# sczhou/CodeFormer

Hardware: NVIDIA H100
Metric: faces_per_sec_512x512_batch32 (higher is better)
Workload: dtype f32 (split-fp16 operands on tensor cores, fp32 accumulate)

## Files before the change

### codeformer_b200/csrc/simt_kernels.cu

```cuda
#include <cuda_fp16.h>
#include <cuda_runtime.h>

#include <atomic>
#include <math.h>
#include <stdint.h>

#include "kernels.cuh"

namespace cfb {

__device__ __forceinline__ float silu_f(float x) { return x / (1.f + expf(-x)); }
__device__ __forceinline__ float gelu_f(float x) { return 0.5f * x * (1.f + erff(x * 0.70710678118654752440f)); }
__device__ __forceinline__ float lrelu_f(float x) { return x > 0.f ? x : 0.2f * x; }

constexpr int CF_BM = 128;
constexpr int CF_BK = 16;
constexpr int CF_APITCH = CF_BM + 4;

template <int BN>
__global__ void __launch_bounds__(256) conv_f32_kernel(ConvArgs a) {
  constexpr int TN = BN / 16;
  __shared__ __align__(16) float As[2][CF_BK][CF_APITCH];
  __shared__ __align__(16) float Bs[2][CF_BK][BN];

  const int t = threadIdx.x;
  const int64_t M = (int64_t)a.N * a.Ho * a.Wo;
  const int64_t m0 = (int64_t)blockIdx.x * CF_BM;
  const int n0 = blockIdx.y * BN;
  const int taps = a.ksize * a.ksize;
  const int kchunks = a.Cin / CF_BK;
  const int nk = taps * kchunks;

  const int arow = t >> 1;
  const int akq = (t & 1) * 8;
  const int64_t am = m0 + arow;
  const bool arow_ok = am < M;
  int an = 0, aoy = 0, aox = 0;
  if (arow_ok) {
    an = (int)(am / ((int64_t)a.Ho * a.Wo));
    int rem = (int)(am - (int64_t)an * a.Ho * a.Wo);
    aoy = rem / a.Wo;
    aox = rem - aoy * a.Wo;
  }
  const float* in_n = a.in + (int64_t)an * a.H * a.W * a.Cin;
  const float* sc_n = a.in_scale ? a.in_scale + (int64_t)an * a.Cin : nullptr;
  const float* sh_n = a.in_shift ? a.in_shift + (int64_t)an * a.Cin : nullptr;

  constexpr int BV = (CF_BK * BN / 4) / 256;
  const int bcol = (BN == 128) ? (t & 31) * 4 : (t & 15) * 4;
  const int brow0 = (BN == 128) ? (t >> 5) : (t >> 4);

  float4 ra[2], rb[BV];

  auto load_global = [&](int it) {
    const int tap = it / kchunks;
    const int c0 = (it - tap * kchunks) * CF_BK;
    int r = 0, s = 0;
    if (a.ksize == 3) { r = tap / 3; s = tap - r * 3; }
    bool ok = arow_ok;
    int iy, ix;
    if (a.mode == CONV_DOWN) {
      iy = aoy * 2 + r; ix = aox * 2 + s;
      ok = ok && iy < a.H && ix < a.W;
    } else if (a.mode == CONV_UP) {
      iy = aoy + r - 1; ix = aox + s - 1;
      ok = ok && iy >= 0 && ix >= 0 && iy < 2 * a.H && ix < 2 * a.W;
      iy >>= 1; ix >>= 1;
    } else {
      const int p = a.ksize >> 1;
      iy = aoy + r - p; ix = aox + s - p;
      ok = ok && iy >= 0 && ix >= 0 && iy < a.H && ix < a.W;
    }
    if (ok) {
      const float* p = in_n + ((int64_t)iy * a.W + ix) * a.Cin + c0 + akq;
      ra[0] = __ldg(reinterpret_cast<const float4*>(p));
      ra[1] = __ldg(reinterpret_cast<const float4*>(p + 4));
      if (sc_n) {
        const float4 s0 = __ldg(reinterpret_cast<const float4*>(sc_n + c0 + akq));
        const float4 s1 = __ldg(reinterpret_cast<const float4*>(sc_n + c0 + akq + 4));
        const float4 h0 = __ldg(reinterpret_cast<const float4*>(sh_n + c0 + akq));
        const float4 h1 = __ldg(reinterpret_cast<const float4*>(sh_n + c0 + akq + 4));
        ra[0].x = fmaf(ra[0].x, s0.x, h0.x); ra[0].y = fmaf(ra[0].y, s0.y, h0.y);
        ra[0].z = fmaf(ra[0].z, s0.z, h0.z); ra[0].w = fmaf(ra[0].w, s0.w, h0.w);
        ra[1].x = fmaf(ra[1].x, s1.x, h1.x); ra[1].y = fmaf(ra[1].y, s1.y, h1.y);
        ra[1].z = fmaf(ra[1].z, s1.z, h1.z); ra[1].w = fmaf(ra[1].w, s1.w, h1.w);
      }
      if (a.in_act == IN_SILU) {
        ra[0].x = silu_f(ra[0].x); ra[0].y = silu_f(ra[0].y); ra[0].z = silu_f(ra[0].z); ra[0].w = silu_f(ra[0].w);
        ra[1].x = silu_f(ra[1].x); ra[1].y = silu_f(ra[1].y); ra[1].z = silu_f(ra[1].z); ra[1].w = silu_f(ra[1].w);
      }
    } else {
      ra[0] = make_float4(0.f, 0.f, 0.f, 0.f);
      ra[1] = ra[0];
    }
    const float* wb = a.wgt_f32 + ((int64_t)tap * a.Cin + c0) * a.Cout + n0 + bcol;
#pragma unroll
    for (int i = 0; i < BV; ++i) {
      const int kr = brow0 + i * 8;
      rb[i] = __ldg(reinterpret_cast<const float4*>(wb + (int64_t)kr * a.Cout));
    }
  };
  auto store_smem = [&](int buf) {
    As[buf][akq + 0][arow] = ra[0].x; As[buf][akq + 1][arow] = ra[0].y;
    As[buf][akq + 2][arow] = ra[0].z; As[buf][akq + 3][arow] = ra[0].w;
    As[buf][akq + 4][arow] = ra[1].x; As[buf][akq + 5][arow] = ra[1].y;
    As[buf][akq + 6][arow] = ra[1].z; As[buf][akq + 7][arow] = ra[1].w;
#pragma unroll
    for (int i = 0; i < BV; ++i) {
      const int kr = brow0 + i * 8;
      *reinterpret_cast<float4*>(&Bs[buf][kr][bcol]) = rb[i];
    }
  };

  const int ty = t >> 4, tx = t & 15;
  float acc[8][TN];
#pragma unroll
  for (int i = 0; i < 8; ++i)
#pragma unroll
    for (int j = 0; j < TN; ++j) acc[i][j] = 0.f;

  load_global(0);
  store_smem(0);
  __syncthreads();
  int buf = 0;
  for (int it = 0; it < nk; ++it) {
    if (it + 1 < nk) load_global(it + 1);
#pragma unroll
    for (int k = 0; k < CF_BK; ++k) {
      const float4 a0 = *reinterpret_cast<const float4*>(&As[buf][k][ty * 4]);
      const float4 a1 = *reinterpret_cast<const float4*>(&As[buf][k][64 + ty * 4]);
      const float av[8] = {a0.x, a0.y, a0.z, a0.w, a1.x, a1.y, a1.z, a1.w};
      float bv[TN];
      {
        const float4 b0 = *reinterpret_cast<const float4*>(&Bs[buf][k][tx * 4]);
        bv[0] = b0.x; bv[1] = b0.y; bv[2] = b0.z; bv[3] = b0.w;
        if (TN == 8) {
          const float4 b1 = *reinterpret_cast<const float4*>(&Bs[buf][k][(BN / 2) + tx * 4]);
          bv[TN - 4] = b1.x; bv[TN - 3] = b1.y; bv[TN - 2] = b1.z; bv[TN - 1] = b1.w;
        }
      }
#pragma unroll
      for (int i = 0; i < 8; ++i)
#pragma unroll
        for (int j = 0; j < TN; ++j) acc[i][j] = fmaf(av[i], bv[j], acc[i][j]);
    }
    if (it + 1 < nk) store_smem(buf ^ 1);
    __syncthreads();
    buf ^= 1;
  }

#pragma unroll
  for (int i = 0; i < 8; ++i) {
    const int64_t m = m0 + ((i < 4) ? (ty * 4 + i) : (64 + ty * 4 + (i - 4)));
    if (m >= M) continue;
#pragma unroll
    for (int h = 0; h < TN / 4; ++h) {
      const int col = n0 + h * (BN / 2) + tx * 4;
      float4 v = make_float4(acc[i][h * 4 + 0], acc[i][h * 4 + 1], acc[i][h * 4 + 2], acc[i][h * 4 + 3]);
      if (a.bias) {
        const float4 b = __ldg(reinterpret_cast<const float4*>(a.bias + col));
        v.x += b.x; v.y += b.y; v.z += b.z; v.w += b.w;
      }
      const int64_t off = m * a.Cout + col;
      if (a.residual) {
        const float4 r = __ldg(reinterpret_cast<const float4*>(a.residual + off));
        v.x += r.x; v.y += r.y; v.z += r.z; v.w += r.w;
      }
      if (a.out_act == OUT_LRELU) {
        v.x = lrelu_f(v.x); v.y = lrelu_f(v.y); v.z = lrelu_f(v.z); v.w = lrelu_f(v.w);
      } else if (a.out_act == OUT_GELU) {
        v.x = gelu_f(v.x); v.y = gelu_f(v.y); v.z = gelu_f(v.z); v.w = gelu_f(v.w);
      }
      if (a.sft_dec) {
        const float4 d = __ldg(reinterpret_cast<const float4*>(a.sft_dec + off));
        const float4 s = __ldg(reinterpret_cast<const float4*>(a.sft_scale + off));
        v.x = d.x + a.sft_w * (d.x * s.x + v.x); v.y = d.y + a.sft_w * (d.y * s.y + v.y);
        v.z = d.z + a.sft_w * (d.z * s.z + v.z); v.w = d.w + a.sft_w * (d.w * s.w + v.w);
      }
      *reinterpret_cast<float4*>(a.out + off) = v;
    }
  }
}

int conv_f32(const ConvArgs& a, cudaStream_t st) {
  CFB_REQUIRE(a.Cin % CF_BK == 0, "conv_f32: Cin must be a multiple of 16");
  CFB_REQUIRE(a.Cout % 64 == 0, "conv_f32: Cout must be a multiple of 64");
  CFB_REQUIRE(a.ksize == 1 || a.ksize == 3, "conv_f32: kernel size must be 1 or 3");
  CFB_REQUIRE(a.wgt_f32 && a.in && a.out, "conv_f32: null tensor");
  const int64_t M = (int64_t)a.N * a.Ho * a.Wo;
  if (M == 0) return 0;
  const unsigned gx = (unsigned)((M + CF_BM - 1) / CF_BM);
  if (a.Cout % 128 == 0) {
    conv_f32_kernel<128><<<dim3(gx, a.Cout / 128), 256, 0, st>>>(a);
  } else {
    conv_f32_kernel<64><<<dim3(gx, a.Cout / 64), 256, 0, st>>>(a);
  }
  CFB_LAUNCH_CHECK();
  return 0;
}

__device__ __forceinline__ float u8_to_model_input(int u) {
  const float t = (float)((double)u / 255.0);
  return __fdiv_rn(__fsub_rn(t, 0.5f), 0.5f);
}
__device__ __forceinline__ unsigned model_output_to_u8(float v) {
  float t = fminf(fmaxf(v, -1.f), 1.f);
  t = __fdiv_rn(__fadd_rn(t, 1.f), 2.f);
  return (unsigned)rintf(__fmul_rn(t, 255.f));
}

template <int COUT, bool U8>
__global__ void __launch_bounds__(256) conv_first_kernel(const float* __restrict__ x, const float* __restrict__ wgt,
                                                         const float* __restrict__ bias, float* __restrict__ out,
                                                         int N, int H, int W, float* __restrict__ gn_part) {
  __shared__ __align__(16) float ws[27 * COUT];
  __shared__ float bs[COUT];
  __shared__ float lut[U8 ? 256 : 1];
  if constexpr (U8) lut[threadIdx.x] = u8_to_model_input(threadIdx.x);
  pdl_launch_dependents();
  pdl_wait();
  for (int i = threadIdx.x; i < 27 * COUT; i += 256) ws[i] = wgt[i];
  for (int i = threadIdx.x; i < COUT; i += 256) bs[i] = bias ? bias[i] : 0.f;
  __syncthreads();
  constexpr int CPT = COUT / 4;
  const int64_t HW = (int64_t)H * W;
  const int64_t quad = (int64_t)blockIdx.x * 64 + (threadIdx.x >> 2);
  const int cg = threadIdx.x & 3;
  const int64_t pix0 = quad * 4;
  if (pix0 >= (int64_t)N * HW) return;
  const int n = (int)(pix0 / HW);
  const int rem = (int)(pix0 - (int64_t)n * HW);
  const int y = rem / W, x0 = rem - y * W;
  float acc[4][CPT];
#pragma unroll
  for (int p = 0; p < 4; ++p)
#pragma unroll
    for (int j = 0; j < CPT; ++j) acc[p][j] = bs[cg * CPT + j];
#pragma unroll
  for (int r = 0; r < 3; ++r) {
    const int iy = y + r - 1;
    const bool rowok = iy >= 0 && iy < H;
#pragma unroll
    for (int c = 0; c < 3; ++c) {
      float v[6];
      if constexpr (U8) {
        const unsigned char* rp8 = reinterpret_cast<const unsigned char*>(x) + ((int64_t)n * HW + (int64_t)iy * W) * 3 + (2 - c);
#pragma unroll
        for (int q = 0; q < 6; ++q) {
          const int ix = x0 + q - 1;
          v[q] = (rowok && ix >= 0 && ix < W) ? lut[__ldg(rp8 + ix * 3)] : 0.f;
        }
      } else {
        const float* rp = x + ((int64_t)n * 3 + c) * HW + (int64_t)iy * W;
#pragma unroll
        for (int q = 0; q < 6; ++q) {
          const int ix = x0 + q - 1;
          v[q] = (rowok && ix >= 0 && ix < W) ? __ldg(rp + ix) : 0.f;
        }
      }
#pragma unroll
      for (int s = 0; s < 3; ++s) {
        const float* wr = ws + ((r * 3 + s) * 3 + c) * COUT + cg * CPT;
#pragma unroll
        for (int j = 0; j < CPT; j += 4) {
          const float4 w4 = *reinterpret_cast<const float4*>(wr + j);
#pragma unroll
          for (int p = 0; p < 4; ++p) {
            acc[p][j] = fmaf(v[p + s], w4.x, acc[p][j]); acc[p][j + 1] = fmaf(v[p + s], w4.y, acc[p][j + 1]);
            acc[p][j + 2] = fmaf(v[p + s], w4.z, acc[p][j + 2]); acc[p][j + 3] = fmaf(v[p + s], w4.w, acc[p][j + 3]);
          }
        }
      }
    }
  }
#pragma unroll
  for (int p = 0; p < 4; ++p) {
    float* o = out + (pix0 + p) * COUT + cg * CPT;
#pragma unroll
    for (int j = 0; j < CPT; j += 4) *reinterpret_cast<float4*>(o + j) = make_float4(acc[p][j], acc[p][j + 1], acc[p][j + 2], acc[p][j + 3]);
  }
  if (gn_part != nullptr) {
    static_assert(COUT == 64, "GroupNorm partials: two channels per group");
    float gs[CPT / 2], gq[CPT / 2];
#pragma unroll
    for (int g = 0; g < CPT / 2; ++g) {
      const float k = acc[0][2 * g];
      float a = 0.f, b = 0.f;
#pragma unroll
      for (int p = 0; p < 4; ++p) {
        const float u = acc[p][2 * g] - k, v = acc[p][2 * g + 1] - k;
        a += u + v;
        b += fmaf(u, u, v * v);
      }
      gn_lane_moments(a, b, k, 8.f);
#pragma unroll
      for (int o = 4, n = 8; o < 32; o <<= 1, n <<= 1) gn_merge_xor(a, b, o, (float)n);
      gs[g] = a; gq[g] = b;
    }
    if ((threadIdx.x & 31) < 4) {
      const int64_t slot = pix0 / 32;
      float2* dst = reinterpret_cast<float2*>(gn_part) + slot * 32 + cg * (CPT / 2);
#pragma unroll
      for (int g = 0; g < CPT / 2; ++g) dst[g] = make_float2(gs[g], gq[g]);
    }
  }
}

int conv_first(const float* x, const float* wgt, const float* bias, float* out, int N, int H, int W, int Cout,
               cudaStream_t st, float* gn_part) {
  CFB_REQUIRE(Cout == 64, "conv_first: only nf=64 is built");
  CFB_REQUIRE(W % 4 == 0, "conv_first: W must be a multiple of 4");
  const int64_t quads = (int64_t)N * H * W / 4;
  if (quads == 0) return 0;
  CFB_REQUIRE(gn_part == nullptr || ((int64_t)H * W) % 256 == 0, "conv_first: GroupNorm partials need H*W % 256 == 0");
  CFB_LAUNCH_PDL((conv_first_kernel<64, false>), dim3((unsigned)((quads + 63) / 64)), dim3(256), 0, st, x, wgt, bias, out, N, H, W, gn_part);
  return 0;
}
int conv_first_u8(const unsigned char* x_bgr_hwc, const float* wgt, const float* bias, float* out, int N, int H, int W,
                  int Cout, cudaStream_t st, float* gn_part) {
  CFB_REQUIRE(Cout == 64, "conv_first: only nf=64 is built");
  CFB_REQUIRE(W % 4 == 0, "conv_first: W must be a multiple of 4");
  const int64_t quads = (int64_t)N * H * W / 4;
  if (quads == 0) return 0;
  CFB_REQUIRE(gn_part == nullptr || ((int64_t)H * W) % 256 == 0, "conv_first: GroupNorm partials need H*W % 256 == 0");
  CFB_LAUNCH_PDL((conv_first_kernel<64, true>), dim3((unsigned)((quads + 63) / 64)), dim3(256), 0, st,
                 reinterpret_cast<const float*>(x_bgr_hwc), wgt, bias, out, N, H, W, gn_part);
  return 0;
}

constexpr int CL_TH = 4, CL_TW = 64;
constexpr int CL_PH = CL_TH + 2, CL_PW = CL_TW + 2;
constexpr int CL_MAX_CIN = 128;
static size_t conv_last_smem(int Cin) { return (size_t)(9 * Cin * 4 + CL_PH * CL_PW * Cin) * sizeof(float); }

template <bool U8>
__global__ void __launch_bounds__(256) conv_last_kernel(const float* __restrict__ in, const float* __restrict__ in_scale,
                                                        const float* __restrict__ in_shift, const float* __restrict__ wgt,
                                                        const float* __restrict__ bias, float* __restrict__ out, int N,
                                                        int H, int W, int Cin) {
  extern __shared__ __align__(16) float sm[];
  float* ws = sm;
  float* xs = ws + 9 * Cin * 4;
  const int Q = Cin / 4;
  const int tiles_x = (W + CL_TW - 1) / CL_TW, tiles_y = (H + CL_TH - 1) / CL_TH;
  const int n = (int)(blockIdx.x / (unsigned)(tiles_x * tiles_y));
  const int trem = (int)blockIdx.x - n * tiles_x * tiles_y;
  const int y0 = (trem / tiles_x) * CL_TH, x0 = (trem % tiles_x) * CL_TW;
  pdl_launch_dependents();
  pdl_wait();
  for (int i = threadIdx.x; i < 9 * Cin; i += 256) {
    ws[i * 4 + 0] = wgt[i * 3 + 0]; ws[i * 4 + 1] = wgt[i * 3 + 1]; ws[i * 4 + 2] = wgt[i * 3 + 2]; ws[i * 4 + 3] = 0.f;
  }
  for (int i = threadIdx.x; i < CL_PH * CL_PW * Q; i += 256) {
    const int q = i % Q, pix = i / Q;
    const int pr = pix / CL_PW, pc = pix - pr * CL_PW;
    const int iy = y0 - 1 + pr, ix = x0 - 1 + pc;
    float4 v = make_float4(0.f, 0.f, 0.f, 0.f);
    if (iy >= 0 && iy < H && ix >= 0 && ix < W) {
      const float4 t = __ldg(reinterpret_cast<const float4*>(in + (((int64_t)n * H + iy) * W + ix) * Cin) + q);
      const float4 s4 = in_scale ? __ldg(reinterpret_cast<const float4*>(in_scale + (int64_t)n * Cin) + q) : make_float4(1.f, 1.f, 1.f, 1.f);
      const float4 h4 = in_shift ? __ldg(reinterpret_cast<const float4*>(in_shift + (int64_t)n * Cin) + q) : make_float4(0.f, 0.f, 0.f, 0.f);
      v = make_float4(fmaf(t.x, s4.x, h4.x), fmaf(t.y, s4.y, h4.y), fmaf(t.z, s4.z, h4.z), fmaf(t.w, s4.w, h4.w));
    }
    reinterpret_cast<float4*>(xs)[pix * Q + (q ^ (pc & 7))] = v;
  }
  __syncthreads();
  const int tr = threadIdx.x / CL_TW, tc = threadIdx.x % CL_TW;
  const int y = y0 + tr, x = x0 + tc;
  float acc[3];
  acc[0] = bias ? bias[0] : 0.f; acc[1] = bias ? bias[1] : 0.f; acc[2] = bias ? bias[2] : 0.f;
  for (int r = 0; r < 3; ++r) {
    const int iy = y + r - 1;
    if (iy < 0 || iy >= H) continue;
    const float4* prow = reinterpret_cast<const float4*>(xs) + (tr + r) * CL_PW * Q;
    for (int c = 0; c < Cin; c += 4) {
      float4 v[3];
#pragma unroll
      for (int s = 0; s < 3; ++s) v[s] = prow[(tc + s) * Q + ((c >> 2) ^ ((tc + s) & 7))];
#pragma unroll
      for (int s = 0; s < 3; ++s) {
        const float* wt = ws + ((r * 3 + s) * Cin + c) * 4;
        const float vj[4] = {v[s].x, v[s].y, v[s].z, v[s].w};
#pragma unroll
        for (int j = 0; j < 4; ++j) {
          const float4 w4 = *reinterpret_cast<const float4*>(wt + j * 4);
          acc[0] = fmaf(vj[j], w4.x, acc[0]);
          acc[1] = fmaf(vj[j], w4.y, acc[1]);
          acc[2] = fmaf(vj[j], w4.z, acc[2]);
        }
      }
    }
  }
  if (y >= H || x >= W) return;
  const int64_t HW = (int64_t)H * W, pix = (int64_t)y * W + x;
  if constexpr (U8) {
    unsigned char* o8 = reinterpret_cast<unsigned char*>(out) + ((int64_t)n * HW + pix) * 3;
    o8[0] = (unsigned char)model_output_to_u8(acc[2]); o8[1] = (unsigned char)model_output_to_u8(acc[1]);
    o8[2] = (unsigned char)model_output_to_u8(acc[0]);
  } else {
    float* o = out + (int64_t)n * 3 * HW + pix;
#pragma unroll
    for (int k = 0; k < 3; ++k) o[k * HW] = acc[k];
  }
}

template <bool U8>
static int launch_conv_last(const float* in, const float* in_scale, const float* in_shift, const float* wgt, const float* bias,
                            float* out, int N, int H, int W, int Cin, cudaStream_t st) {
  CFB_REQUIRE(Cin % 32 == 0 && Cin <= CL_MAX_CIN, "conv_last: Cin must be a multiple of 32 and at most 128");
  if (N == 0 || H == 0 || W == 0) return 0;
  static std::atomic<uint64_t> attr_done{0};
  int dev = 0;
  CFB_CUDA(cudaGetDevice(&dev));
  const uint64_t bit = 1ull << (dev & 63);
  if (!(attr_done.load(std::memory_order_acquire) & bit)) {
    CFB_CUDA(cudaFuncSetAttribute(conv_last_kernel<U8>, cudaFuncAttributeMaxDynamicSharedMemorySize, (int)conv_last_smem(CL_MAX_CIN)));
    attr_done.fetch_or(bit, std::memory_order_release);
  }
  const int64_t tiles = (int64_t)N * ((H + CL_TH - 1) / CL_TH) * ((W + CL_TW - 1) / CL_TW);
  CFB_REQUIRE(tiles <= 0x7fffffffLL, "conv_last: too many tiles");
  CFB_LAUNCH_PDL(conv_last_kernel<U8>, dim3((unsigned)tiles), dim3(256), conv_last_smem(Cin), st, in, in_scale, in_shift, wgt, bias,
                 out, N, H, W, Cin);
  return 0;
}

int conv_last(const float* in, const float* in_scale, const float* in_shift, const float* wgt, const float* bias,
              float* out, int N, int H, int W, int Cin, cudaStream_t st) {
  return launch_conv_last<false>(in, in_scale, in_shift, wgt, bias, out, N, H, W, Cin, st);
}
int conv_last_u8(const float* in, const float* in_scale, const float* in_shift, const float* wgt, const float* bias,
                 unsigned char* out_bgr_hwc, int N, int H, int W, int Cin, cudaStream_t st) {
  return launch_conv_last<true>(in, in_scale, in_shift, wgt, bias, reinterpret_cast<float*>(out_bgr_hwc), N, H, W, Cin, st);
}

__global__ void u8_to_input_kernel(const unsigned char* __restrict__ img, float* __restrict__ x, int64_t HW, int64_t total) {
  for (int64_t i = (int64_t)blockIdx.x * blockDim.x + threadIdx.x; i < total; i += (int64_t)gridDim.x * blockDim.x) {
    const int64_t n = i / (3 * HW);
    const int64_t r = i - n * 3 * HW;
    const int c = (int)(r / HW);
    const int64_t px = r - (int64_t)c * HW;
    x[i] = u8_to_model_input(img[(n * HW + px) * 3 + (2 - c)]);
  }
}
__global__ void output_to_u8_kernel(const float* __restrict__ x, unsigned char* __restrict__ img, int64_t HW, int64_t total) {
  for (int64_t i = (int64_t)blockIdx.x * blockDim.x + threadIdx.x; i < total; i += (int64_t)gridDim.x * blockDim.x) {
    const int64_t n = i / (3 * HW);
    const int64_t r = i - n * 3 * HW;
    const int64_t px = r / 3;
    const int k = (int)(r - px * 3);
    img[i] = (unsigned char)model_output_to_u8(x[(n * 3 + (2 - k)) * HW + px]);
  }
}
int u8_to_input(const unsigned char* img_bgr_hwc, float* x_nchw, int N, int64_t HW, cudaStream_t st) {
  const int64_t total = (int64_t)N * 3 * HW;
  if (total == 0) return 0;
  u8_to_input_kernel<<<(unsigned)((total + 255) / 256 > 148 * 16 ? 148 * 16 : (total + 255) / 256), 256, 0, st>>>(img_bgr_hwc, x_nchw, HW, total);
  CFB_LAUNCH_CHECK();
  return 0;
}
int output_to_u8(const float* x_nchw, unsigned char* img_bgr_hwc, int N, int64_t HW, cudaStream_t st) {
  const int64_t total = (int64_t)N * 3 * HW;
  if (total == 0) return 0;
  output_to_u8_kernel<<<(unsigned)((total + 255) / 256 > 148 * 16 ? 148 * 16 : (total + 255) / 256), 256, 0, st>>>(x_nchw, img_bgr_hwc, HW, total);
  CFB_LAUNCH_CHECK();
  return 0;
}

__global__ void relayout_oihw_kernel(const float* __restrict__ w, float* __restrict__ out, int Cout, int Cin, int k) {
  const int64_t total = (int64_t)Cout * Cin * k * k;
  for (int64_t i = (int64_t)blockIdx.x * blockDim.x + threadIdx.x; i < total; i += (int64_t)gridDim.x * blockDim.x) {
    const int co = (int)(i % Cout);
    const int ci = (int)((i / Cout) % Cin);
    const int tap = (int)(i / ((int64_t)Cout * Cin));
    out[i] = w[((int64_t)co * Cin + ci) * k * k + tap];
  }
}
int relayout_oihw_to_tck(const float* oihw, float* out, int Cout, int Cin, int k, cudaStream_t st) {
  const int64_t total = (int64_t)Cout * Cin * k * k;
  relayout_oihw_kernel<<<(unsigned)((total + 255) / 256 > 4096 ? 4096 : (total + 255) / 256), 256, 0, st>>>(oihw, out, Cout,
                                                                                                          Cin, k);
  CFB_LAUNCH_CHECK();
  return 0;
}

static inline int gn_chunk_pixels(int HW) { return HW < 2048 ? HW : 2048; }
size_t gn_workspace_bytes(int N, int HW, int C) {
  const int chunks = HW / gn_chunk_pixels(HW);
  return (size_t)N * chunks * 32 * 2 * sizeof(double);
}

__global__ void __launch_bounds__(256) gn_partial_kernel(const float* __restrict__ x, double* __restrict__ part, int HW,
                                                         int C, int CP, int groups) {
  __shared__ double ssum[256 * 4];
  __shared__ double ssq[256 * 4];
  __shared__ double csum[1024];
  __shared__ double csq[1024];
  const int t = threadIdx.x;
  const int C4 = C >> 2;
  const int PL = 256 / C4;
  const int c4 = t % C4, pl = t / C4;
  const int chunk = blockIdx.x, n = blockIdx.y, chunks = gridDim.x;
  const float* base = x + ((int64_t)n * HW + (int64_t)chunk * CP) * C + c4 * 4;
  double s[4] = {0.0, 0.0, 0.0, 0.0}, q[4] = {0.0, 0.0, 0.0, 0.0};
  for (int p = pl; p < CP; p += PL) {
    const float4 v = __ldg(reinterpret_cast<const float4*>(base + (int64_t)p * C));
    const double a = v.x, b = v.y, c = v.z, d = v.w;
    s[0] += a; s[1] += b; s[2] += c; s[3] += d;
    q[0] = fma(a, a, q[0]); q[1] = fma(b, b, q[1]); q[2] = fma(c, c, q[2]); q[3] = fma(d, d, q[3]);
  }
#pragma unroll
  for (int j = 0; j < 4; ++j) { ssum[pl * C + c4 * 4 + j] = s[j]; ssq[pl * C + c4 * 4 + j] = q[j]; }
  __syncthreads();
  for (int c = t; c < C; c += 256) {
    double a = 0.0, b = 0.0;
    for (int l = 0; l < PL; ++l) { a += ssum[l * C + c]; b += ssq[l * C + c]; }
    csum[c] = a; csq[c] = b;
  }
  __syncthreads();
  if (t < groups) {
    const int cpg = C / groups;
    double a = 0.0, b = 0.0;
    for (int c = 0; c < cpg; ++c) { a += csum[t * cpg + c]; b += csq[t * cpg + c]; }
    double* o = part + (((int64_t)n * chunks + chunk) * groups + t) * 2;
    o[0] = a; o[1] = b;
  }
}

__global__ void gn_final_kernel(const double* __restrict__ part, const float* __restrict__ gamma,
                                const float* __restrict__ beta, float* __restrict__ scale, float* __restrict__ shift,
                                int HW, int C, int chunks, int groups, float eps) {
  __shared__ double gmean[64], grstd[64];
  const int n = blockIdx.x, t = threadIdx.x;
  const int cpg = C / groups;
  if (t < groups) {
    double a = 0.0, b = 0.0;
    for (int k = 0; k < chunks; ++k) {
      const double* p = part + (((int64_t)n * chunks + k) * groups + t) * 2;
      a += p[0]; b += p[1];
    }
    const double cnt = (double)HW * cpg;
    const double mean = a / cnt;
    double var = b / cnt - mean * mean;
    if (var < 0.0) var = 0.0;
    gmean[t] = mean;
    grstd[t] = 1.0 / sqrt(var + (double)eps);
  }
  __syncthreads();
  for (int c = t; c < C; c += blockDim.x) {
    const int g = c / cpg;
    const double sc = grstd[g] * (double)gamma[c];
    scale[(int64_t)n * C + c] = (float)sc;
    shift[(int64_t)n * C + c] = (float)((double)beta[c] - gmean[g] * sc);
  }
}

int gn_coef(const float* x, const float* gamma, const float* beta, float* scale, float* shift, int N, int HW, int C,
            int groups, float eps, void* ws, cudaStream_t st) {
  CFB_REQUIRE(C % 4 == 0 && (C / 4) <= 256 && 256 % (C / 4) == 0, "gn_coef: C must be 4*divisor of 256");
  CFB_REQUIRE(groups <= 64 && C % groups == 0, "gn_coef: bad group count");
  const int CP = gn_chunk_pixels(HW);
  CFB_REQUIRE(HW % CP == 0, "gn_coef: H*W must be a multiple of the chunk size");
  if (N == 0) return 0;
  const int chunks = HW / CP;
  gn_partial_kernel<<<dim3(chunks, N), 256, 0, st>>>(x, (double*)ws, HW, C, CP, groups);
  CFB_LAUNCH_CHECK();
  gn_final_kernel<<<N, 256, 0, st>>>((const double*)ws, gamma, beta, scale, shift, HW, C, chunks, groups, eps);
  CFB_LAUNCH_CHECK();
  return 0;
}

__host__ __device__ inline int gn_final_split(int slots) {
  int g = slots / 256;
  return g < 1 ? 1 : (g > 16 ? 16 : g);
}
__global__ void __launch_bounds__(256) gn_final_f32_kernel(const float* __restrict__ part, const float* __restrict__ gamma,
                                                           const float* __restrict__ beta, float* __restrict__ scale,
                                                           float* __restrict__ shift, int HW, int C, int slots, float eps,
                                                           double* __restrict__ part2, unsigned* __restrict__ counters) {
  __shared__ double ps[8][33], pq[8][33];
  __shared__ double gmean[32], grstd[32];
  __shared__ int is_last;
  pdl_launch_dependents();
  pdl_wait();
  const int n = blockIdx.y, G = gridDim.x, blk = blockIdx.x, t = threadIdx.x;
  const int g = t & 31, stripe = t >> 5;
  const int per = (slots + G - 1) / G;
  const int lo = blk * per, hi = min(slots, lo + per);
  const int cpg = C / 32;
  const float2* base = reinterpret_cast<const float2*>(part) + (int64_t)n * slots * 32 + g;
  const double K = (double)__ldg(base).x, m = (double)HW * cpg / slots;
  double a = 0.0, b = 0.0;
  int k = lo + stripe;
  for (; k + 24 < hi; k += 32) {
    const float2 v0 = __ldg(base + (int64_t)k * 32), v1 = __ldg(base + (int64_t)(k + 8) * 32);
    const float2 v2 = __ldg(base + (int64_t)(k + 16) * 32), v3 = __ldg(base + (int64_t)(k + 24) * 32);
    const double d0 = (double)v0.x - K, d1 = (double)v1.x - K, d2 = (double)v2.x - K, d3 = (double)v3.x - K;
    a += (d0 + d1) + (d2 + d3);
    b += (fma(m * d0, d0, (double)v0.y) + fma(m * d1, d1, (double)v1.y)) + (fma(m * d2, d2, (double)v2.y) + fma(m * d3, d3, (double)v3.y));
  }
  for (; k < hi; k += 8) {
    const float2 v = __ldg(base + (int64_t)k * 32);
    const double d = (double)v.x - K;
    a += d; b += fma(m * d, d, (double)v.y);
  }
  ps[stripe][g] = a; pq[stripe][g] = b;
  __syncthreads();
  double sa = 0.0, sb = 0.0;
  if (t < 32) {
    for (int s = 0; s < 8; ++s) { sa += ps[s][t]; sb += pq[s][t]; }
  }
  if (G > 1) {
    if (t < 32) {
      double* dst = part2 + ((int64_t)n * G + blk) * 64;
      dst[2 * t] = sa; dst[2 * t + 1] = sb;
      __threadfence();
    }
    __syncthreads();
    if (t == 0) is_last = (atomicAdd(counters + n, 1u) == (unsigned)(G - 1));
    __syncthreads();
    if (!is_last) return;
    __threadfence();
    if (t < 32) {
      sa = 0.0; sb = 0.0;
      const double* src = part2 + (int64_t)n * G * 64;
      for (int q = 0; q < G; ++q) { sa += __ldcg(src + q * 64 + 2 * t); sb += __ldcg(src + q * 64 + 2 * t + 1); }
    }
    if (t == 0) counters[n] = 0u;
  }
  if (t < 32) {
    const double dm = sa / slots;
    double var = sb / ((double)HW * cpg) - dm * dm;
    if (var < 0.0) var = 0.0;
    gmean[t] = K + dm;
    grstd[t] = 1.0 / sqrt(var + (double)eps);
  }
  __syncthreads();
  for (int c = t; c < C; c += 256) {
    const int gg = c / cpg;
    const double sc = grstd[gg] * (double)gamma[c];
    scale[(int64_t)n * C + c] = (float)sc;
    shift[(int64_t)n * C + c] = (float)((double)beta[c] - gmean[gg] * sc);
  }
}
size_t gn_final_scratch_bytes(int N, int slots) {
  const int G = gn_final_split(slots);
  return G > 1 ? (size_t)N * G * 64 * sizeof(double) : 0;
}
int gn_coef_from_partials(const float* part, int slots, const float* gamma, const float* beta, float* scale, float* shift,
                          int N, int HW, int C, int groups, float eps, void* scratch, unsigned* counters, cudaStream_t st) {
  CFB_REQUIRE(groups == 32 && C % 32 == 0, "gn_coef_from_partials: 32 groups only");
  CFB_REQUIRE(slots > 0 && (int64_t)slots * 32 == HW, "gn_coef_from_partials: a slot holds 32 pixels of the image");
  if (N == 0) return 0;
  const int G = gn_final_split(slots);
  CFB_REQUIRE(G == 1 || (scratch && counters), "gn_coef_from_partials: scratch / counters missing");
  CFB_REQUIRE(N <= 65535, "gn_coef_from_partials: batch too large");
  CFB_LAUNCH_PDL(gn_final_f32_kernel, dim3(G, N), dim3(256), 0, st, part, gamma, beta, scale, shift, HW, C, slots, eps, (double*)scratch,
                 counters);
  return 0;
}

__global__ void gn_cat_partials_kernel(const float2* __restrict__ a, const float2* __restrict__ b, float2* __restrict__ out,
                                       int64_t total, float half_cnt) {
  pdl_launch_dependents();
  pdl_wait();
  for (int64_t i = (int64_t)blockIdx.x * blockDim.x + threadIdx.x; i < total; i += (int64_t)gridDim.x * blockDim.x) {
    const int g = (int)(i & 31);
    const int64_t slot = i >> 5;
    const float2* src = (g < 16) ? a + slot * 32 + 2 * g : b + slot * 32 + 2 * (g - 16);
    const float2 u = __ldg(src), v = __ldg(src + 1);
    const float d = u.x - v.x;
    out[i] = make_float2(0.5f * (u.x + v.x), (u.y + v.y) + (d * d) * half_cnt);
  }
}
int gn_cat_partials(const float* a_part, const float* b_part, float* out_part, int64_t total_slots, int C, cudaStream_t st) {
  CFB_REQUIRE(C % 32 == 0, "gn_cat_partials: 32 groups of C channels");
  const int64_t total = total_slots * 32;
  if (total == 0) return 0;
  const int64_t blocks = (total + 255) / 256;
  CFB_LAUNCH_PDL(gn_cat_partials_kernel, dim3((unsigned)(blocks > 2048 ? 2048 : blocks)), dim3(256), 0, st, (const float2*)a_part,
                 (const float2*)b_part, (float2*)out_part, total, 0.5f * (float)C);
  return 0;
}

__global__ void affine_act_kernel(const float4* __restrict__ x, const float* __restrict__ scale,
                                  const float* __restrict__ shift, float4* __restrict__ y, int64_t total4, int64_t HWC4,
                                  int C, int act) {
  for (int64_t i = (int64_t)blockIdx.x * blockDim.x + threadIdx.x; i < total4; i += (int64_t)gridDim.x * blockDim.x) {
    const int n = (int)(i / HWC4);
    const int c = (int)((i * 4) % C);
    float4 v = __ldg(x + i);
    if (scale) {
      const float4 s = __ldg(reinterpret_cast<const float4*>(scale + (int64_t)n * C + c));
      const float4 h = __ldg(reinterpret_cast<const float4*>(shift + (int64_t)n * C + c));
      v.x = fmaf(v.x, s.x, h.x); v.y = fmaf(v.y, s.y, h.y); v.z = fmaf(v.z, s.z, h.z); v.w = fmaf(v.w, s.w, h.w);
    }
    if (act == IN_SILU) { v.x = silu_f(v.x); v.y = silu_f(v.y); v.z = silu_f(v.z); v.w = silu_f(v.w); }
    y[i] = v;
  }
}
int affine_act(const float* x, const float* scale, const float* shift, float* y, int N, int HW, int C, int act,
               cudaStream_t st) {
  CFB_REQUIRE(C % 4 == 0, "affine_act: C must be a multiple of 4");
  const int64_t total4 = (int64_t)N * HW * C / 4;
  if (total4 == 0) return 0;
  const int64_t blocks = (total4 + 255) / 256;
  affine_act_kernel<<<(unsigned)(blocks > 148 * 16 ? 148 * 16 : blocks), 256, 0, st>>>(
      (const float4*)x, scale, shift, (float4*)y, total4, (int64_t)HW * C / 4, C, act);
  CFB_LAUNCH_CHECK();
  return 0;
}

__device__ __forceinline__ void split_store4(__half* __restrict__ hi, __half* __restrict__ lo, int64_t off, const float4& o);

constexpr int AT_S = 256;
constexpr int AT_QB = 32;

template <int D>
__global__ void __launch_bounds__(256) attention_kernel(const float* __restrict__ q, const float* __restrict__ k,
                                                        const float* __restrict__ v, float* __restrict__ out, int q_pitch,
                                                        int k_pitch, int v_pitch, int o_pitch, float scale,
                                                        __half* __restrict__ out_hi, __half* __restrict__ out_lo) {
  extern __shared__ __align__(16) float sm[];
  float* Qs = sm;
  float* Ks = Qs + 32 * AT_QB;
// ... 1012 lines not shown
```

Baseline: 174.6.

## Stage conv_first output through shared memory and async-load conv_last input tile

conv_first now writes its per-thread results into a swizzled per-warp shared-memory stage and then emits fully coalesced float4 stores for 32 contiguous pixels. This replaces the old strided per-thread stores. conv_last loads its input halo tile with cp.async zero-fill, overlaps that with the weight and scale/shift loads, and applies the GroupNorm affine in place in shared memory. It also gains a parameterised pixels-per-thread path, which is set to 1 here. The cost is much more dynamic shared memory for conv_first, which lowers occupancy, plus extra synchronisation and a second pass over the tile.

```diff
diff --git a/codeformer_b200/csrc/simt_kernels.cu b/codeformer_b200/csrc/simt_kernels.cu
--- a/codeformer_b200/csrc/simt_kernels.cu
+++ b/codeformer_b200/csrc/simt_kernels.cu
@@ -209,13 +209,18 @@
   return (unsigned)rintf(__fmul_rn(t, 255.f));
 }
 
+constexpr int CFIRST_COUT = 64;
+static size_t conv_first_smem() { return (size_t)(27 * CFIRST_COUT + CFIRST_COUT + 256 + 8 * 32 * CFIRST_COUT) * sizeof(float); }
+
 template <int COUT, bool U8>
-__global__ void __launch_bounds__(256) conv_first_kernel(const float* __restrict__ x, const float* __restrict__ wgt,
+__global__ void __launch_bounds__(256, U8 ? 1 : 2) conv_first_kernel(const float* __restrict__ x, const float* __restrict__ wgt,
                                                          const float* __restrict__ bias, float* __restrict__ out,
                                                          int N, int H, int W, float* __restrict__ gn_part) {
-  __shared__ __align__(16) float ws[27 * COUT];
-  __shared__ float bs[COUT];
-  __shared__ float lut[U8 ? 256 : 1];
+  extern __shared__ __align__(16) float fsm[];
+  float* ws = fsm;
+  float* bs = ws + 27 * COUT;
+  float* lut = bs + COUT;
+  float4* stage = reinterpret_cast<float4*>(lut + 256) + (threadIdx.x >> 5) * 32 * (COUT / 4);
   if constexpr (U8) lut[threadIdx.x] = u8_to_model_input(threadIdx.x);
   pdl_launch_dependents();
   pdl_wait();
@@ -223,14 +228,16 @@
   for (int i = threadIdx.x; i < COUT; i += 256) bs[i] = bias ? bias[i] : 0.f;
   __syncthreads();
   constexpr int CPT = COUT / 4;
-  const int64_t HW = (int64_t)H * W;
+  const int64_t HW = (int64_t)H * W, NHW = (int64_t)N * HW;
   const int64_t quad = (int64_t)blockIdx.x * 64 + (threadIdx.x >> 2);
   const int cg = threadIdx.x & 3;
   const int64_t pix0 = quad * 4;
-  if (pix0 >= (int64_t)N * HW) return;
-  const int n = (int)(pix0 / HW);
-  const int rem = (int)(pix0 - (int64_t)n * HW);
-  const int y = rem / W, x0 = rem - y * W;
+  const int64_t wpix0 = ((int64_t)blockIdx.x * 256 + (threadIdx.x & ~31));
+  if (wpix0 >= NHW) return;
+  const bool valid = pix0 < NHW;
+  const int n = valid ? (int)(pix0 / HW) : 0;
+  const int rem = valid ? (int)(pix0 - (int64_t)n * HW) : 0;
+  const int y = valid ? rem / W : -2, x0 = rem - (valid ? y * W : 0);
   float acc[4][CPT];
 #pragma unroll
   for (int p = 0; p < 4; ++p)
@@ -273,12 +280,29 @@
       }
     }
   }
-#pragma unroll
-  for (int p = 0; p < 4; ++p) {
-    float* o = out + (pix0 + p) * COUT + cg * CPT;
-#pragma unroll
-    for (int j = 0; j < CPT; j += 4) *reinterpret_cast<float4*>(o + j) = make_float4(acc[p][j], acc[p][j + 1], acc[p][j + 2], acc[p][j + 3]);
-  }
+  static_assert(COUT == 64, "output stage: 16 channel quads per pixel");
+  {
+    const int qi = (threadIdx.x & 31) >> 2;
+#pragma unroll
+    for (int p = 0; p < 4; ++p) {
+      const int px = qi * 4 + p;
+#pragma unroll
+      for (int j = 0; j < CPT; j += 4) {
+        const int cq = cg * (CPT / 4) + j / 4;
+        stage[px * (COUT / 4) + (cq ^ (((cq >> 3) & 1) | (((px >> 2) & 1) << 1)))] =
+            make_float4(acc[p][j], acc[p][j + 1], acc[p][j + 2], acc[p][j + 3]);
+      }
+    }
+    __syncwarp();
+    const int lane = threadIdx.x & 31;
+    float4* o = reinterpret_cast<float4*>(out + wpix0 * COUT);
+#pragma unroll 4
+    for (int i = lane; i < 32 * (COUT / 4); i += 32) {
+      const int px = i / (COUT / 4), cq = i % (COUT / 4);
+      if (wpix0 + px < NHW) o[i] = stage[px * (COUT / 4) + (cq ^ (((cq >> 3) & 1) | (((px >> 2) & 1) << 1)))];
+    }
+  }
+  if (!valid) return;
   if (gn_part != nullptr) {
     static_assert(COUT == 64, "GroupNorm partials: two channels per group");
     float gs[CPT / 2], gq[CPT / 2];
@@ -306,41 +330,61 @@
   }
 }
 
-int conv_first(const float* x, const float* wgt, const float* bias, float* out, int N, int H, int W, int Cout,
-               cudaStream_t st, float* gn_part) {
-  CFB_REQUIRE(Cout == 64, "conv_first: only nf=64 is built");
+template <typename K>
+static int allow_dynamic_smem(K kernel, size_t bytes, std::atomic<uint64_t>& done) {
+  int dev = 0;
+  CFB_CUDA(cudaGetDevice(&dev));
+  const uint64_t bit = 1ull << (dev & 63);
+  if (!(done.load(std::memory_order_acquire) & bit)) {
+    CFB_CUDA(cudaFuncSetAttribute(kernel, cudaFuncAttributeMaxDynamicSharedMemorySize, (int)bytes));
+    done.fetch_or(bit, std::memory_order_release);
+  }
+  return 0;
+}
+
+template <bool U8>
+static int launch_conv_first(const float* x, const float* wgt, const float* bias, float* out, int N, int H, int W, int Cout,
+                             cudaStream_t st, float* gn_part) {
+  CFB_REQUIRE(Cout == CFIRST_COUT, "conv_first: only nf=64 is built");
   CFB_REQUIRE(W % 4 == 0, "conv_first: W must be a multiple of 4");
   const int64_t quads = (int64_t)N * H * W / 4;
   if (quads == 0) return 0;
   CFB_REQUIRE(gn_part == nullptr || ((int64_t)H * W) % 256 == 0, "conv_first: GroupNorm partials need H*W % 256 == 0");
-  CFB_LAUNCH_PDL((conv_first_kernel<64, false>), dim3((unsigned)((quads + 63) / 64)), dim3(256), 0, st, x, wgt, bias, out, N, H, W, gn_part);
-  return 0;
+  static std::atomic<uint64_t> attr_done{0};
+  CFB_CHECK(allow_dynamic_smem(conv_first_kernel<CFIRST_COUT, U8>, conv_first_smem(), attr_done));
+  CFB_LAUNCH_PDL((conv_first_kernel<CFIRST_COUT, U8>), dim3((unsigned)((quads + 63) / 64)), dim3(256), conv_first_smem(), st, x, wgt,
+                 bias, out, N, H, W, gn_part);
+  return 0;
+}
+int conv_first(const float* x, const float* wgt, const float* bias, float* out, int N, int H, int W, int Cout,
+               cudaStream_t st, float* gn_part) {
+  return launch_conv_first<false>(x, wgt, bias, out, N, H, W, Cout, st, gn_part);
 }
 int conv_first_u8(const unsigned char* x_bgr_hwc, const float* wgt, const float* bias, float* out, int N, int H, int W,
                   int Cout, cudaStream_t st, float* gn_part) {
-  CFB_REQUIRE(Cout == 64, "conv_first: only nf=64 is built");
-  CFB_REQUIRE(W % 4 == 0, "conv_first: W must be a multiple of 4");
-  const int64_t quads = (int64_t)N * H * W / 4;
-  if (quads == 0) return 0;
-  CFB_REQUIRE(gn_part == nullptr || ((int64_t)H * W) % 256 == 0, "conv_first: GroupNorm partials need H*W % 256 == 0");
-  CFB_LAUNCH_PDL((conv_first_kernel<64, true>), dim3((unsigned)((quads + 63) / 64)), dim3(256), 0, st,
-                 reinterpret_cast<const float*>(x_bgr_hwc), wgt, bias, out, N, H, W, gn_part);
-  return 0;
-}
-
-constexpr int CL_TH = 4, CL_TW = 64;
+  return launch_conv_first<true>(reinterpret_cast<const float*>(x_bgr_hwc), wgt, bias, out, N, H, W, Cout, st, gn_part);
+}
+
+constexpr int CL_TH = 4, CL_TW = 64, CL_PX = 1;
+constexpr int CL_THREADS = CL_TH * CL_TW / CL_PX;
 constexpr int CL_PH = CL_TH + 2, CL_PW = CL_TW + 2;
 constexpr int CL_MAX_CIN = 128;
-static size_t conv_last_smem(int Cin) { return (size_t)(9 * Cin * 4 + CL_PH * CL_PW * Cin) * sizeof(float); }
+static size_t conv_last_smem(int Cin) { return (size_t)(9 * Cin * 4 + 2 * Cin + CL_PH * CL_PW * Cin) * sizeof(float); }
+
+__device__ __forceinline__ void cp_async16_zfill(void* dst, const void* src, bool valid) {
+  const unsigned d = (unsigned)__cvta_generic_to_shared(dst);
+  asm volatile("cp.async.cg.shared.global [%0], [%1], 16, %2;" ::"r"(d), "l"(src), "r"(valid ? 16 : 0) : "memory");
+}
 
 template <bool U8>
-__global__ void __launch_bounds__(256) conv_last_kernel(const float* __restrict__ in, const float* __restrict__ in_scale,
-                                                        const float* __restrict__ in_shift, const float* __restrict__ wgt,
-                                                        const float* __restrict__ bias, float* __restrict__ out, int N,
-                                                        int H, int W, int Cin) {
+__global__ void __launch_bounds__(CL_THREADS) conv_last_kernel(const float* __restrict__ in, const float* __restrict__ in_scale,
+                                                               const float* __restrict__ in_shift, const float* __restrict__ wgt,
+                                                               const float* __restrict__ bias, float* __restrict__ out, int N,
+                                                               int H, int W, int Cin) {
   extern __shared__ __align__(16) float sm[];
   float* ws = sm;
-  float* xs = ws + 9 * Cin * 4;
+  float* ss = ws + 9 * Cin * 4;
+  float* xs = ss + 2 * Cin;
   const int Q = Cin / 4;
   const int tiles_x = (W + CL_TW - 1) / CL_TW, tiles_y = (H + CL_TH - 1) / CL_TH;
   const int n = (int)(blockIdx.x / (unsigned)(tiles_x * tiles_y));
@@ -348,59 +392,84 @@
   const int y0 = (trem / tiles_x) * CL_TH, x0 = (trem % tiles_x) * CL_TW;
   pdl_launch_dependents();
   pdl_wait();
-  for (int i = threadIdx.x; i < 9 * Cin; i += 256) {
-    ws[i * 4 + 0] = wgt[i * 3 + 0]; ws[i * 4 + 1] = wgt[i * 3 + 1]; ws[i * 4 + 2] = wgt[i * 3 + 2]; ws[i * 4 + 3] = 0.f;
-  }
-  for (int i = threadIdx.x; i < CL_PH * CL_PW * Q; i += 256) {
+  for (int i = threadIdx.x; i < CL_PH * CL_PW * Q; i += CL_THREADS) {
     const int q = i % Q, pix = i / Q;
     const int pr = pix / CL_PW, pc = pix - pr * CL_PW;
     const int iy = y0 - 1 + pr, ix = x0 - 1 + pc;
-    float4 v = make_float4(0.f, 0.f, 0.f, 0.f);
-    if (iy >= 0 && iy < H && ix >= 0 && ix < W) {
-      const float4 t = __ldg(reinterpret_cast<const float4*>(in + (((int64_t)n * H + iy) * W + ix) * Cin) + q);
-      const float4 s4 = in_scale ? __ldg(reinterpret_cast<const float4*>(in_scale + (int64_t)n * Cin) + q) : make_float4(1.f, 1.f, 1.f, 1.f);
-      const float4 h4 = in_shift ? __ldg(reinterpret_cast<const float4*>(in_shift + (int64_t)n * Cin) + q) : make_float4(0.f, 0.f, 0.f, 0.f);
-      v = make_float4(fmaf(t.x, s4.x, h4.x), fmaf(t.y, s4.y, h4.y), fmaf(t.z, s4.z, h4.z), fmaf(t.w, s4.w, h4.w));
-    }
-    reinterpret_cast<float4*>(xs)[pix * Q + (q ^ (pc & 7))] = v;
-  }
-  __syncthreads();
-  const int tr = threadIdx.x / CL_TW, tc = threadIdx.x % CL_TW;
+    const bool ok = iy >= 0 && iy < H && ix >= 0 && ix < W;
+    const float* src = ok ? in + (((int64_t)n * H + iy) * W + ix) * Cin + q * 4 : in;
+    cp_async16_zfill(reinterpret_cast<float4*>(xs) + pix * Q + (q ^ ((pc / CL_PX) & 7)), src, ok);
+  }
+  asm volatile("cp.async.commit_group;" ::: "memory");
+  for (int i = threadIdx.x; i < 9 * Cin; i += CL_THREADS) {
+    ws[i * 4 + 0] = wgt[i * 3 + 0]; ws[i * 4 + 1] = wgt[i * 3 + 1]; ws[i * 4 + 2] = wgt[i * 3 + 2]; ws[i * 4 + 3] = 0.f;
+  }
+  for (int c = threadIdx.x; c < Cin; c += CL_THREADS) {
+    ss[c] = in_scale ? in_scale[(int64_t)n * Cin + c] : 1.f;
+    ss[Cin + c] = in_shift ? in_shift[(int64_t)n * Cin + c] : 0.f;
+  }
+  asm volatile("cp.async.wait_group 0;" ::: "memory");
+  __syncthreads();
+  for (int i = threadIdx.x; i < CL_PH * CL_PW * Q; i += CL_THREADS) {
+    const int q = i % Q, pix = i / Q;
+    const int pr = pix / CL_PW, pc = pix - pr * CL_PW;
+    const int iy = y0 - 1 + pr, ix = x0 - 1 + pc;
+    if (iy < 0 || iy >= H || ix < 0 || ix >= W) continue;
+    float4* p = reinterpret_cast<float4*>(xs) + pix * Q + (q ^ ((pc / CL_PX) & 7));
+    const float4 t = *p;
+    const float4 s4 = reinterpret_cast<const float4*>(ss)[q], h4 = reinterpret_cast<const float4*>(ss + Cin)[q];
+    *p = make_float4(fmaf(t.x, s4.x, h4.x), fmaf(t.y, s4.y, h4.y), fmaf(t.z, s4.z, h4.z), fmaf(t.w, s4.w, h4.w));
+  }
+  __syncthreads();
+  const int tr = threadIdx.x / (CL_TW / CL_PX), tc = (threadIdx.x % (CL_TW / CL_PX)) * CL_PX;
   const int y = y0 + tr, x = x0 + tc;
-  float acc[3];
-  acc[0] = bias ? bias[0] : 0.f; acc[1] = bias ? bias[1] : 0.f; acc[2] = bias ? bias[2] : 0.f;
+  float acc[CL_PX][3];
+#pragma unroll
+  for (int p = 0; p < CL_PX; ++p) {
+    acc[p][0] = bias ? bias[0] : 0.f; acc[p][1] = bias ? bias[1] : 0.f; acc[p][2] = bias ? bias[2] : 0.f;
+  }
   for (int r = 0; r < 3; ++r) {
     const int iy = y + r - 1;
     if (iy < 0 || iy >= H) continue;
     const float4* prow = reinterpret_cast<const float4*>(xs) + (tr + r) * CL_PW * Q;
+#pragma unroll 2
     for (int c = 0; c < Cin; c += 4) {
-      float4 v[3];
-#pragma unroll
-      for (int s = 0; s < 3; ++s) v[s] = prow[(tc + s) * Q + ((c >> 2) ^ ((tc + s) & 7))];
+      float4 v[CL_PX + 2];
+#pragma unroll
+      for (int s = 0; s < CL_PX + 2; ++s) v[s] = prow[(tc + s) * Q + ((c >> 2) ^ (((tc + s) / CL_PX) & 7))];
 #pragma unroll
       for (int s = 0; s < 3; ++s) {
         const float* wt = ws + ((r * 3 + s) * Cin + c) * 4;
-        const float vj[4] = {v[s].x, v[s].y, v[s].z, v[s].w};
 #pragma unroll
         for (int j = 0; j < 4; ++j) {
           const float4 w4 = *reinterpret_cast<const float4*>(wt + j * 4);
-          acc[0] = fmaf(vj[j], w4.x, acc[0]);
-          acc[1] = fmaf(vj[j], w4.y, acc[1]);
-          acc[2] = fmaf(vj[j], w4.z, acc[2]);
+#pragma unroll
+          for (int p = 0; p < CL_PX; ++p) {
+            const float4 vp = v[p + s];
+            const float vj = j == 0 ? vp.x : j == 1 ? vp.y : j == 2 ? vp.z : vp.w;
+            acc[p][0] = fmaf(vj, w4.x, acc[p][0]);
+            acc[p][1] = fmaf(vj, w4.y, acc[p][1]);
+            acc[p][2] = fmaf(vj, w4.z, acc[p][2]);
+          }
         }
       }
     }
   }
-  if (y >= H || x >= W) return;
-  const int64_t HW = (int64_t)H * W, pix = (int64_t)y * W + x;
-  if constexpr (U8) {
-    unsigned char* o8 = reinterpret_cast<unsigned char*>(out) + ((int64_t)n * HW + pix) * 3;
-    o8[0] = (unsigned char)model_output_to_u8(acc[2]); o8[1] = (unsigned char)model_output_to_u8(acc[1]);
-    o8[2] = (unsigned char)model_output_to_u8(acc[0]);
-  } else {
-    float* o = out + (int64_t)n * 3 * HW + pix;
-#pragma unroll
-    for (int k = 0; k < 3; ++k) o[k * HW] = acc[k];
+  if (y >= H) return;
+  const int64_t HW = (int64_t)H * W;
+#pragma unroll
+  for (int p = 0; p < CL_PX; ++p) {
+    if (x + p >= W) break;
+    const int64_t pix = (int64_t)y * W + x + p;
+    if constexpr (U8) {
+      unsigned char* o8 = reinterpret_cast<unsigned char*>(out) + ((int64_t)n * HW + pix) * 3;
+      o8[0] = (unsigned char)model_output_to_u8(acc[p][2]); o8[1] = (unsigned char)model_output_to_u8(acc[p][1]);
+      o8[2] = (unsigned char)model_output_to_u8(acc[p][0]);
+    } else {
+      float* o = out + (int64_t)n * 3 * HW + pix;
+#pragma unroll
+      for (int k = 0; k < 3; ++k) o[k * HW] = acc[p][k];
+    }
   }
 }
 
@@ -410,16 +479,10 @@
   CFB_REQUIRE(Cin % 32 == 0 && Cin <= CL_MAX_CIN, "conv_last: Cin must be a multiple of 32 and at most 128");
   if (N == 0 || H == 0 || W == 0) return 0;
   static std::atomic<uint64_t> attr_done{0};
-  int dev = 0;
-  CFB_CUDA(cudaGetDevice(&dev));
-  const uint64_t bit = 1ull << (dev & 63);
-  if (!(attr_done.load(std::memory_order_acquire) & bit)) {
-    CFB_CUDA(cudaFuncSetAttribute(conv_last_kernel<U8>, cudaFuncAttributeMaxDynamicSharedMemorySize, (int)conv_last_smem(CL_MAX_CIN)));
-    attr_done.fetch_or(bit, std::memory_order_release);
-  }
+  CFB_CHECK(allow_dynamic_smem(conv_last_kernel<U8>, conv_last_smem(CL_MAX_CIN), attr_done));
   const int64_t tiles = (int64_t)N * ((H + CL_TH - 1) / CL_TH) * ((W + CL_TW - 1) / CL_TW);
   CFB_REQUIRE(tiles <= 0x7fffffffLL, "conv_last: too many tiles");
-  CFB_LAUNCH_PDL(conv_last_kernel<U8>, dim3((unsigned)tiles), dim3(256), conv_last_smem(Cin), st, in, in_scale, in_shift, wgt, bias,
+  CFB_LAUNCH_PDL(conv_last_kernel<U8>, dim3((unsigned)tiles), dim3(CL_THREADS), conv_last_smem(Cin), st, in, in_scale, in_shift, wgt, bias,
                  out, N, H, W, Cin);
   return 0;
 }
```

Result: no change. 175.4, median of 6 (+0.5%).
